# cyberlife-coder/velesdb

Measured on AMD Instinct MI355X. Metric: qps_at_recall10_1Mx768_k10, higher is better.
Workload: dtype f32; 1 GPU; 1000000x768 f32 cosine, k=10, exact distance sweep + fused GPU top-k (BASELINE configs[1]); 1024 queries/step, 1024 queries per corpus pass (sweep_topk_gemm_bf16_pp<dot, WIDE> over normalised bf16 images of rows and queries (cosine; ping-po; rows=1000000, dim=768, k=10, parallelism=replicas x1 (query stream split, no collective)

## Files before the change

velesdb_amd/csrc/select_stage.hip:

```cpp
#include <algorithm>
#include <array>
#include <cstdio>
#include <cstdlib>
#include <cstring>
#include <string>
#include <vector>

#include "vdb_probe_env.hpp"
#include "vdb_select_stage.hpp"
#include "vdb_wide.hpp"

namespace vdb {

static inline uint32_t opt_max_tile(const vdb_hip_index* ix) { return (uint32_t)opt_value(ix, VDB_OPT_MAX_QUERY_TILE); }
static inline int opt_engine(const vdb_hip_index* ix) { return (int)opt_value(ix, VDB_OPT_SWEEP_ENGINE); }
static inline int opt_selector(const vdb_hip_index* ix) { return (int)opt_value(ix, VDB_OPT_SELECTOR_LEVEL); }
static const bool g_bf16_seed = [] {
  const char* e = probe_env("VELESDB_BF16_SEED");
  return !(e && e[0] == '0');
}();
static const bool g_pool_select = [] {
  const char* e = probe_env("VELESDB_POOL_SELECT");
  return !(e && e[0] == '0');
}();
// ... 721 lines not shown
      launch_merge(true, mg, kFallbackGatherMax, st);
      ag.qcount = qcount;
      ag.qcount_max = kFallbackGatherMax;
    }
    if (!gather_all) {
      ag.part_keys = ix->s_fb_keys.as<uint64_t>();
      ag.n_rows = n;
      ag.rows = ix->rows.as<float>();
      e = launch_sweep_gemm(ix->metric, fp, ag, st, tile_needed);
      if (e != hipSuccess) return fail(VDB_ERR_HIP, std::string("exact fallback launch: ") + hipGetErrorString(e));
      MergeArgs mf{};
      mf.part_keys = ag.part_keys;
      mf.ext_ids = ix->ext_ids.as<uint64_t>();
      mf.out_ids = reinterpret_cast<uint64_t*>(sd + o_fid);
      mf.out_scores = reinterpret_cast<float*>(sd + o_fsc);
      mf.out_n = reinterpret_cast<uint32_t*>(sd + o_fn);
      mf.n_lists = fp.G;
      mf.k = k;
      mf.gate = flags;
      if (gather_ok) {
        mf.skip_cnt = qcount;
        mf.skip_le = kFallbackGatherMax;
      }
      launch_merge(true, mf, nqg, st);
      fin.fb_ids = mf.out_ids;
      fin.fb_scores = mf.out_scores;
      fin.fb_n = mf.out_n;
    }
    if (gather_ok) {
      fin.max_listed = gather_all ? 0u : kFallbackGatherMax;
      fin.g_ids = mg.out_ids;
      fin.g_scores = mg.out_scores;
      fin.g_n = mg.out_n;
    }
    launch_select_finish(fin, st);
  }
  ix->split_flags_off = o_flags;
  ix->split_flags_n = nqg;
  ix->split_flags_stream = st;
  if (ev) (void)hipEventRecord(ev->b, st);
  VDB_HIP(hipGetLastError());
  return VDB_OK;
}


static const bool g_wide_small_k = [] {
  const char* e = probe_env("VELESDB_WIDE_SMALL_K");
  return !(e && e[0] == '0');
}();
static const bool g_wide_fuse = [] {
  const char* e = probe_env("VELESDB_WIDE_FUSE");
  return !(e && e[0] == '0');
}();
int select_level_wide(vdb_hip_index* ix, uint32_t nq_left, uint32_t k, bool sq8) {
  if (opt_selector(ix) < 2 || (!sq8 && opt_engine(ix) != 1) || opt_max_tile(ix) < 128) return 0;
  if (ix->metric != VDB_COSINE && ix->metric != VDB_DOT && (sq8 || ix->metric != VDB_EUCLIDEAN)) return 0;
  if (ix->dim % 64 != 0 || ix->dim < 128 || ix->row_stride != ix->dim) return 0;
  if (k == 0 || k > kWideMaxK || ix->n_rows < kGemmBf16MinRows || ix->n_rows >= 0xFFFFFF00ull) return 0;
  if (k <= kGemmBf16MaxK && (opt_selector(ix) < 3 || !g_wide_small_k)) return 0;
  if (!sq8 && ix->metric != VDB_EUCLIDEAN && sweep_mfma_lds_bytes(1, k, ix->dim) > 160 * 1024) return 0;
  if (!sq8 && ix->metric == VDB_EUCLIDEAN && !l2_gather_fits(ix->dim, k)) return 0;
  if (!select_chunk(nq_left, sq8 ? kSelectMinQueriesSq8 : 0)) return 0;
  if (ix->sel_stats && ix->sel_stats[2] != ix->sel_seq_seen) {
    ix->sel_seq_seen = ix->sel_stats[2];
    if (ix->sel_stats[3] == 4u && (uint64_t)ix->sel_stats[0] * 16 > ix->sel_stats[1]) ix->wide_hold = 64;
  }
  if (ix->wide_hold) {
    ix->wide_hold--;
    return 0;
  }
  return 4;
}

int32_t brute_wide_dev(vdb_hip_index* ix, const float* d_q, uint64_t q_stride, uint32_t nqg, uint32_t k, uint64_t* d_ids, float* d_scores,
                       uint32_t* d_n, hipStream_t st, bool sq8) {
  const bool cosn = !sq8 && cosine_normalised(ix);
  const bool l2 = !sq8 && ix->metric == VDB_EUCLIDEAN;
  const int sel_metric = (cosn || l2) ? VDB_DOT : ix->metric;
  int32_t rc = sq8 ? ensure_sq8_select(ix, st) : (l2 ? ensure_l2_select(ix, st) : (cosn ? ensure_cosn(ix, st) : ensure_sel16(ix, st)));
  if (rc != VDB_OK) return rc;
  const uint32_t dim_a = ix->dim + 64, dim_s = ix->dim + 4;
  const uint16_t* img_rows = sq8 ? ix->sq8_img.as<uint16_t>()
                                 : (l2 ? ix->l2_img.as<uint16_t>() : (cosn ? ix->cosn_img.as<uint16_t>() : ix->rows_bf16.as<uint16_t>()));
  const uint64_t img_stride = l2 ? (uint64_t)dim_a : ((cosn || sq8) ? (uint64_t)ix->dim : ix->bf16_stride);
  const DevBuf& rho_buf = sq8 ? ix->sq8_rho : (l2 ? ix->l2_rho : (cosn ? ix->cosn_rho : ix->bf16_rho));
  const float* sel_norms = sq8 ? ix->sq8_nrm.as<float>() : ix->norms.as<float>();
  DevBuf& list_buf = sq8 ? ix->s_part_cnt : ix->s_fb_keys;
  const uint32_t sel_dim = l2 ? dim_a : ix->dim;
  ix->last_select_level = 4;
  ix->last_kernels |= VDB_KERNEL_SELECT_BF16;
  const uint8_t* alive = ix->any_dead ? ix->alive.as<uint8_t>() : nullptr;
  const uint32_t n = (uint32_t)ix->n_rows, dim = ix->dim;
  static const uint32_t g_small_seed_rows = [] {
    const char* e = probe_env("VELESDB_WIDE_SEED_ROWS");
    const long v = e ? atol(e) : 0;
    return v >= 1024 && v <= (long)kWideSeedRows ? (uint32_t)v / 256u * 256u : kSplitSeedRows;
  }();
  const uint32_t R0 = std::min<uint32_t>(k <= kWideSmallSeedMaxK ? g_small_seed_rows : kWideSeedRows, n), ngrp = (R0 + 15) / 16;
  GemmSchedule sch;
  {
    static const std::array<uint32_t, 3> mult = [] {
      std::array<uint32_t, 3> m{1, 4, 16};
      if (const char* e = probe_env("VELESDB_WIDE_STEPS")) {
        unsigned a = 0, b = 0, c = 0;
        const int got = sscanf(e, "%u,%u,%u", &a, &b, &c);
        m = {got >= 1 ? a : 0u, got >= 2 ? b : 0u, got >= 3 ? c : 0u};
      }
      return m;
    }();
    const uint32_t head[3] = {mult[0], mult[1], mult[2]};
    gemm_schedule(nqg, 0, n, ix->n_cus, head, 0, &sch);
  }
  int g_nqt = 3;
  while (g_nqt > 1 && sweep_mfma_lds_bytes(g_nqt, k, dim) > 160 * 1024) g_nqt--;
  const int g_waves = g_nqt >= 2 ? kMfmaWaves2 : kMfmaWaves1;
  const uint32_t g_B = l2 ? 8u : (uint32_t)g_nqt * 16;
  const uint32_t ntiles16 = (n + 15) / 16;
  const int g_blocks = l2 ? blocks_for(ix, 8, (n + 7) / 8)
                          : (int)std::max<int64_t>(1, std::min<int64_t>(((int64_t)ntiles16 + g_waves - 1) / g_waves, (int64_t)ix->n_cus));
  size_t off = 0;
  auto take = [&](size_t bytes) {
    const size_t o = off;
    off = (off + bytes + 15) & ~(size_t)15;
    return o;
  };
  const size_t o_tau = take((size_t)nqg * 8), o_delta = take((size_t)nqg * 4), o_qn = take((size_t)nqg * 4), o_rho = take((size_t)nqg * 4),
               o_cnt = take((size_t)nqg * 4), o_state = take((size_t)nqg * 4), o_flags = take((size_t)nqg * 4 + 16), o_qmap = take((size_t)nqg * 8),
               o_gid = take((size_t)nqg * k * 8), o_gsc = take((size_t)nqg * k * 4), o_gn = take((size_t)nqg * 4), o_nmax = take(16),
               o_extra = take((size_t)nqg * 4);
  hipError_t e;
  if ((e = ix->s_seed.reserve(off, false, st)) != hipSuccess || (e = list_buf.reserve((size_t)nqg * kWideCap * 8, false, st)) != hipSuccess ||
      (e = ix->s_part_keys.reserve((size_t)nqg * ngrp * 8, false, st)) != hipSuccess ||
      (!sq8 && (e = ix->s_part_cnt.reserve((size_t)nqg * g_blocks * k * 8, false, st)) != hipSuccess) ||
      (e = ix->s_misc.reserve(((size_t)nqg + 256) * img_stride * 2 + (l2 ? (size_t)nqg * dim_s * 4 + 16 : 0), false, st)) != hipSuccess)
    return fail(VDB_ERR_OOM, "wide selection scratch");
  unsigned char* sd = ix->s_seed.as<unsigned char>();
  uint16_t* q16 = ix->s_misc.as<uint16_t>();
  float* qnorms = reinterpret_cast<float*>(sd + o_qn);
  float* rho_q = rho_buf.p ? reinterpret_cast<float*>(sd + o_rho) : nullptr;
  uint32_t* flags = reinterpret_cast<uint32_t*>(sd + o_flags);
  uint32_t* qcount = flags + nqg;
  uint32_t* qmap = reinterpret_cast<uint32_t*>(sd + o_qmap);
  uint32_t* qslot = qmap + nqg;
  uint32_t* norm_max = reinterpret_cast<uint32_t*>(sd + o_nmax);
  EventPair* ev = next_events(ix);
  if (ev) (void)hipEventRecord(ev->a, st);
  if (l2) {
    float* qaug = reinterpret_cast<float*>(ix->s_misc.as<unsigned char>() + ((((size_t)nqg + 256) * img_stride * 2 + 15) & ~(size_t)15));
    launch_l2_augment_queries(d_q, q_stride, q16, dim_a, qaug, dim_s, nqg, dim, st);
    if (rho_q) launch_query_round_error(d_q, q_stride, rho_q, nqg, dim, st);
    PrepArgs pq{};
    pq.rows = d_q;
    pq.norms = qnorms;
    pq.row_stride = q_stride;
    pq.n_rows = nqg;
    pq.dim = dim;
    pq.words = ix->words;
    launch_prep_rows(pq, st);
    VDB_HIP(hipMemsetAsync(flags, 0, (size_t)nqg * 4 + 16, st));
  } else if (cosn) launch_seln_prep_queries(d_q, q_stride, q16, img_stride, qnorms, rho_q, flags, nqg + 4, nqg, dim, st);
  else launch_sel16_prep_queries(d_q, q_stride, q16, img_stride, qnorms, rho_q, flags, nqg + 4, nqg, dim, st);
  if (nqg % 256u) VDB_HIP(hipMemsetAsync(q16 + (size_t)nqg * img_stride, 0, (size_t)256 * img_stride * 2, st));
  if (ix->metric == VDB_DOT || l2) launch_max_norm(sel_norms, n, norm_max, st);
  WideArgs wa{};
  wa.keys = list_buf.as<uint64_t>();
  wa.eps_extra = sq8 ? 1.5e-4f : 0.0f;
  wa.cnt = reinterpret_cast<uint32_t*>(sd + o_cnt);
  wa.state = reinterpret_cast<uint32_t*>(sd + o_state);
  wa.tau = reinterpret_cast<uint64_t*>(sd + o_tau);
  wa.delta = reinterpret_cast<float*>(sd + o_delta);
  wa.qnorms = qnorms;
  wa.rho_q = rho_q;
  wa.rho_max_bits = rho_q ? rho_buf.as<uint32_t>() : nullptr;
  wa.norm_max_bits = norm_max;
  wa.extra = l2 ? reinterpret_cast<float*>(sd + o_extra) : nullptr;
  wa.cap = kWideCap;
  wa.k = k;
  wa.dim = dim;
  launch_seed_scores_bf16(sel_metric, img_rows, img_stride, sel_norms, alive, q16, img_stride, qnorms, ix->s_part_keys.as<uint64_t>(), R0,
                          nqg, sel_dim, st);
  if (l2) launch_wide_seed_l2(wa, ix->s_part_keys.as<uint64_t>(), ngrp, dim_a, nqg, st);
  else launch_wide_seed(ix->metric, wa, ix->s_part_keys.as<uint64_t>(), ngrp, nqg, st);
  for (int j = 0; j < sch.n_launch; j++) {
    EventPair* evs = next_sel_events(ix);
    if (evs) (void)hipEventRecord(evs->a, st);
    e = launch_sweep_gemm_bf16_wide(sel_metric, sch.bp[j], img_rows, img_stride, sel_norms, alive, q16, img_stride, wa.tau, wa.keys, wa.cnt,
                                    wa.cap, sel_dim, nqg, st, qnorms);
    if (evs) (void)hipEventRecord(evs->b, st);
    if (e != hipSuccess) return fail(VDB_ERR_HIP, std::string("wide selection launch: ") + hipGetErrorString(e));
    if (j + 1 < sch.n_launch || l2 || sq8 || !g_wide_fuse) launch_wide_reseed(wa, nqg, st);
  }
  WideOutArgs wo{};
  wo.rows = ix->rows.as<float>();
  wo.norms = ix->norms.as<float>();
  wo.queries = d_q;
  wo.ext_ids = ix->ext_ids.as<uint64_t>();
  wo.out_ids = d_ids;
  wo.out_scores = d_scores;
  wo.out_n = d_n;
  wo.flags = flags;
  wo.qcount = qcount;
  wo.qmap = qmap;
  wo.qslot = qslot;
  wo.row_stride = ix->row_stride;
  wo.q_stride = q_stride;
  wo.dim_pad = (dim + 127) / 128 * 128;
  if (sq8) {
    wo.sq8_codes = ix->sq8_codes.as<uint8_t>();
    wo.sq8_min = ix->sq8_min.as<float>();
    wo.sq8_max = ix->sq8_max.as<float>();
    wo.sq8_nsq = ix->sq8_nsq.as<float>();
    wo.sq8_stride = ix->sq8_stride;
    launch_wide_rerank_sq8(ix->metric, wa, wo, nqg, st);
    SelectFinishArgs fq{};
    fq.flags = flags;
    fq.qcount = qcount;
    fq.qslot = qslot;
    fq.out_ids = d_ids;
    fq.out_scores = d_scores;
    fq.out_n = d_n;
    fq.nq = nqg;
    fq.k = k;
    if (ix->sel_stats) {
      fq.stats_host = ix->sel_stats;
      fq.stats_seq = ++ix->sel_seq;
      fq.stats_level = 4u;
    }
    const int32_t rf = sq8_fallback_flagged(ix, d_q, q_stride, nqg, k, qmap, fq, st);
    if (rf != VDB_OK) return rf;
    ix->split_flags_off = o_flags;
    ix->split_flags_n = nqg;
    ix->split_flags_stream = st;
    if (ev) (void)hipEventRecord(ev->b, st);
    VDB_HIP(hipGetLastError());
    return VDB_OK;
  }
  static const bool g_wide_stamps = [] {
    const char* e = probe_env("VELESDB_WIDE_STAMPS");
    return e && e[0] == '1';
  }();
// ... 90 lines not shown
```

velesdb_amd/csrc/sweep_gemm_bf16.hip:

```cpp
#include <algorithm>

#include "vdb_probe_env.hpp"
#include "vdb_device.hpp"
#include "vdb_kernels.hpp"

namespace vdb {

typedef float f32x4 __attribute__((ext_vector_type(4)));
typedef __bf16 bf16x8 __attribute__((ext_vector_type(8)));
typedef __attribute__((address_space(3))) void* lds_ptr_t;
typedef __attribute__((address_space(3))) uint32_t lds_u32_t;

constexpr int kG16BM = 256, kG16BN = 256, kG16Waves = 8;
constexpr int kG16Cap = 12;
constexpr int kG16Queue = 39;
#ifndef VDB_G16_DUMP_MAX_LANES
#define VDB_G16_DUMP_MAX_LANES 6
#endif
constexpr int kG16DumpMaxLanes = VDB_G16_DUMP_MAX_LANES;
static_assert(kG16Queue == 39, "g16_protocol.inc keeps two hot lanes' 64 accumulators in queue entries 8 .. 39");
static_assert(kG16Queue <= 64 && kG16Queue >= 32, "the finish pass takes one queue entry per lane; one hot lane's 32 elements fit");
constexpr size_t kOffCand = 131072, kOffTauk = kOffCand + (size_t)kG16BN * kG16Cap * 8, kOffCnts = kOffTauk + kG16BN * 8,
                 kOffQn = kOffCnts + kG16BN * 4, kOffVns = kOffQn + kG16BN * 4, kOffFlags = kOffVns + kG16BM * 4,
                 kOffQueue = kOffFlags + 16,
                 kQueueBytes = 368,
                
                 kG16Lds = kOffQueue + kG16Waves * kQueueBytes;
static_assert(kG16Lds <= 160 * 1024, "LDS budget");
static_assert((size_t)(kG16Queue + 1) * 8 + kG16Queue + 4 <= 364 + 4 && (size_t)(kG16Queue + 1) * 8 + kG16Queue <= 364, "queue layout");

struct Bf16GemmArgs {
  const uint16_t* rows;
  const float* norms;
  const uint8_t* alive;
  const uint16_t* queries;
  const uint64_t* tau0;
  uint64_t* part_keys;
  uint64_t row_stride, q_stride;
  uint32_t n_rows, dim, nq, k;
  uint32_t KT, G, nqt, qper;
  uint32_t row_tile0;
  uint32_t list_stride, list_off;
  const float* qnorms;
  uint64_t* blk_tau;
  const float* qnorms_half;
  unsigned long long* dbg;
  uint64_t* wide_keys;
  uint32_t* wide_cnt;
  uint32_t wide_cap;
};

__device__ __forceinline__ uint32_t lane_now() {
  uint32_t l;
  asm volatile("v_mbcnt_lo_u32_b32 %0, -1, 0\n\tv_mbcnt_hi_u32_b32 %0, -1, %0" : "=v"(l));
  return l;
}

__device__ __forceinline__ void mfma_bf16_inplace(f32x4& c, const f32x4& a, const f32x4& b) {
  asm volatile("v_mfma_f32_16x16x32_bf16 %0, %1, %2, %0" : "+v"(c) : "v"(a), "v"(b));
}
__device__ __forceinline__ void mfma_bf16_first(f32x4& c, const f32x4& a, const f32x4& b) {
  asm volatile("v_mfma_f32_16x16x32_bf16 %0, %1, %2, 0" : "=&v"(c) : "v"(a), "v"(b));
}
__device__ __forceinline__ void mfma_drain() { asm volatile("s_nop 15\n\ts_nop 15" ::: "memory"); }

typedef int i32x4 __attribute__((ext_vector_type(4)));
__device__ __forceinline__ void glds_b128(const i32x4& rsrc, uint32_t voff, uint32_t soff, uint32_t lds_addr) {
  asm volatile("s_mov_b32 m0, %3\n\ts_nop 3\n\tbuffer_load_dwordx4 %0, %1, %2 offen lds"
               :
               : "v"(voff), "s"(rsrc), "s"(soff), "s"(lds_addr)
               : "m0");
}
__device__ __forceinline__ i32x4 make_rsrc(const void* base, uint32_t num_records = 0x7FFFFFFFu) {
  const uint64_t b = reinterpret_cast<uint64_t>(base);
  return i32x4{(int)(uint32_t)b, (int)((uint32_t)(b >> 32) & 0xFFFFu), (int)num_records, 0x00020000};
}
__device__ __forceinline__ i32x4 make_rsrc_uniform(const void* base, uint32_t num_records = 0x7FFFFFFFu) {
  const uint64_t b = reinterpret_cast<uint64_t>(base);
  const uint32_t lo = (uint32_t)__builtin_amdgcn_readfirstlane((int)(uint32_t)b);
  const uint32_t hi = (uint32_t)__builtin_amdgcn_readfirstlane((int)(uint32_t)(b >> 32));
  return i32x4{(int)lo, (int)(hi & 0xFFFFu), __builtin_amdgcn_readfirstlane((int)num_records), 0x00020000};
}
__device__ __forceinline__ uint32_t a_tile_records(uint32_t n_rows, uint32_t rt, uint32_t kt, uint64_t row_stride) {
  const uint64_t left = (uint64_t)(n_rows - rt * (uint32_t)kG16BM) * row_stride * 2u - (uint64_t)kt * 128u;
  return (uint32_t)(left < 0x7FFFFFFFull ? left : 0x7FFFFFFFull);
}
__device__ __forceinline__ uint32_t norm_records(uint32_t n_rows, uint32_t rt) {
  return min(n_rows - rt * (uint32_t)kG16BM, (uint32_t)kG16BM) * 4u;
}
__device__ __forceinline__ void wait_glds() { asm volatile("s_waitcnt vmcnt(0)" ::: "memory"); }

template <int METRIC, bool SPLIT>
__global__ __launch_bounds__(512, 2) void sweep_topk_gemm_bf16_glds(Bf16GemmArgs a) {
  constexpr bool HIB = true;
  constexpr bool WIDE = false;
  constexpr int BM = kG16BM, BN = kG16BN, WAVES = kG16Waves, CAP = kG16Cap, QCAP = kG16Queue;
  extern __shared__ __attribute__((aligned(16))) unsigned char smem[];
  uint64_t* cand = reinterpret_cast<uint64_t*>(smem + kOffCand);
  uint64_t* tauk = reinterpret_cast<uint64_t*>(smem + kOffTauk);
  uint32_t* cnts = reinterpret_cast<uint32_t*>(smem + kOffCnts);
  float* qn = reinterpret_cast<float*>(smem + kOffQn);
  float* vns = reinterpret_cast<float*>(smem + kOffVns);
// ... 162 lines not shown
  __syncthreads();
  for (uint32_t rt = rt_first; rt < ntiles; rt += a.G) {
    VDB_G16_STEP(0, true);
    __syncthreads();
    for (uint32_t kt = 1; kt + 1 < a.KT; kt++) {
      VDB_G16_STEP(kt, false);
      __syncthreads();
    }
    VDB_G16_STEP(a.KT - 1, false);
    const bool more = it < total;
#define VDB_G16_ACC_F(V) (V)
#include "g16_quicktest.inc"
    if constexpr (METRIC == kHamming || METRIC == kJaccard) {
#include "g16_quicktest_bits.inc"
    } else {
#include "g16_quicktest_dense.inc"
    }
#define VDB_G16_ACC_ELEM(X, A) asm volatile("v_mov_b32 %0, %1" : "=v"(X) : "v"(A))
#define VDB_G16_NO_DUMP 1
#include "g16_protocol.inc"
#undef VDB_G16_NO_DUMP
#undef VDB_G16_ACC_ELEM
#undef VDB_G16_ACC_F
  }
#undef VDB_G16_STEP
#undef VDB_G16_ADVANCE
#undef VDB_G16_GLDS
#undef VDB_G16_REQ
#include "g16_writeout.inc"
}

template <bool FP4>
__device__ __forceinline__ void mfma_accv(f32x4& c, const f32x4& a, const f32x4& b) {
  if (FP4)
    asm volatile("v_mfma_scale_f32_16x16x128_f8f6f4 %0, %1, %2, %0, %3, %3 op_sel_hi:[0,0,0] cbsz:4 blgp:4" : "+v"(c) : "v"(a), "v"(b), "v"(0x7F7F7F7Fu));
  else
    asm volatile("v_mfma_f32_16x16x32_bf16 %0, %1, %2, %0" : "+v"(c) : "v"(a), "v"(b));
}
template <bool FP4>
__device__ __forceinline__ void mfma_accv_first(f32x4& c, const f32x4& a, const f32x4& b) {
  if (FP4)
    asm volatile("v_mfma_scale_f32_16x16x128_f8f6f4 %0, %1, %2, 0, %3, %3 op_sel_hi:[0,0,0] cbsz:4 blgp:4" : "=&v"(c) : "v"(a), "v"(b), "v"(0x7F7F7F7Fu));
  else
    asm volatile("v_mfma_f32_16x16x32_bf16 %0, %1, %2, 0" : "=&v"(c) : "v"(a), "v"(b));
}
template <int OFF>
__device__ __forceinline__ void lds_frag_read(f32x4& dst, uint32_t addr) {
  asm volatile("ds_read_b128 %0, %1 offset:%2" : "=v"(dst) : "v"(addr), "n"(OFF));
}
__device__ __forceinline__ void pp_barrier_reads_done() { asm volatile("s_waitcnt lgkmcnt(0)\n\ts_barrier" ::: "memory"); }
__device__ __forceinline__ void pp_barrier() { asm volatile("s_barrier" ::: "memory"); }
__device__ __forceinline__ void pp_wait_dma6() { asm volatile("s_waitcnt vmcnt(6)" ::: "memory"); }

template <int METRIC, bool FP4 = false, bool WIDE = false>
__global__ __launch_bounds__(512, 2) void sweep_topk_gemm_bf16_pp(Bf16GemmArgs a) {
  static_assert(FP4 == (METRIC == kHamming || METRIC == kJaccard), "the four-bit instance serves the bit metrics, the bf16 instance Cosine / DotProduct");
  constexpr bool HIB = METRIC != kHamming;
  constexpr int BM = kG16BM, BN = kG16BN, WAVES = kG16Waves, CAP = kG16Cap, QCAP = kG16Queue;
  extern __shared__ __attribute__((aligned(16))) unsigned char smem[];
  uint64_t* cand = reinterpret_cast<uint64_t*>(smem + kOffCand);
  uint64_t* tauk = reinterpret_cast<uint64_t*>(smem + kOffTauk);
  uint32_t* cnts = reinterpret_cast<uint32_t*>(smem + kOffCnts);
  float* qn = reinterpret_cast<float*>(smem + kOffQn);
  float* vns = reinterpret_cast<float*>(smem + kOffVns);
  volatile lds_u32_t* flags = (volatile lds_u32_t*)(lds_ptr_t)(smem + kOffFlags);

  const int tid = (int)threadIdx.x;
  const int lane = tid & 63;
  const int wib = __builtin_amdgcn_readfirstlane(tid >> 6);
  const int wr = wib >> 2, wq = wib & 3;
  uint64_t* wq_keys = reinterpret_cast<uint64_t*>(smem + kOffQueue + (size_t)wib * kQueueBytes);
  uint8_t* wq_qs = reinterpret_cast<uint8_t*>(wq_keys + QCAP + 1);

  const uint32_t bid = blockIdx.x;
  const uint32_t xcd = bid & 7u, slot_id = bid >> 3;
  const uint32_t qt = slot_id % a.nqt;
  const uint32_t g = (slot_id / a.nqt) * 8u + xcd;
  const uint32_t q0 = qt * a.qper;
  const uint32_t nq_t = min(a.qper, a.nq - q0);
  const uint32_t k = a.k;
  const uint16_t* queries = a.queries + (size_t)q0 * a.q_stride;

  if (tid < BN) {
    cnts[tid] = 0;
    tauk[tid] = ((uint32_t)tid < nq_t && a.tau0) ? a.tau0[q0 + tid] : kKeyInvalid;
    qn[tid] = 0.0f;
  }
  if (tid < 4) flags[tid] = 0u;
  __syncthreads();
  if (a.qnorms) {
    if ((uint32_t)tid < nq_t) qn[tid] = a.qnorms[q0 + tid];
  } else if (a.qnorms_half) {
    if ((uint32_t)tid < nq_t) qn[tid] = a.qnorms_half[q0 + tid];
  } else {
    for (uint32_t b = wib; b < nq_t; b += WAVES) {
      const uint16_t* qp = queries + (size_t)b * a.q_stride;
      float nacc = 0.0f;
      for (uint32_t c = lane; c * 4 < a.dim; c += 64)
#pragma unroll
        for (int e = 0; e < 4; e++) {
          const uint32_t i = c * 4 + e;
          if (i < a.dim) {
            const float x = __uint_as_float((uint32_t)qp[i] << 16);
            nacc = __builtin_fmaf(x, x, nacc);
          }
        }
// ... 85 lines not shown
    } \
  } while (0)
  uint32_t c = 0;
  if (total) {
    VDB_PP_REQ_A(0, rt_first, 0, 0);
    VDB_PP_REQ_A(1, rt_first, 0, 0);
    VDB_PP_REQ_B(0, 0, 0);
    VDB_PP_REQ_B(1, 0, 0);
    VDB_PP_NEXT2();
    VDB_PP_REQ_B(0, kt2, 1);
    VDB_PP_REQ_A(0, rt2, kt2, 1);
    VDB_PP_REQ_A(1, rt2, kt2, 1);
    VDB_PP_NEXT2();
    pp_wait_dma6();
  }
  pp_barrier();
  if (total) VDB_PP_READ_A(a0v, 0, 0);
  if (wr == 1) pp_barrier();
#ifndef VDB_PP_STAMP
#define VDB_PP_STAMP 0
#endif
#ifndef VDB_PP_STAMP_METRIC
#define VDB_PP_STAMP_METRIC kCosine
#endif
#if VDB_PP_STAMP
  const bool st_on = a.dbg != nullptr && blockIdx.x == 8u && (wib == 0 || wib == 4) && METRIC == VDB_PP_STAMP_METRIC;
  uint32_t st_acc[28] = {0, 0, 0, 0, 0, 0, 0, 0, 0, 0, 0, 0, 0, 0, 0, 0, 0, 0, 0, 0, 0, 0, 0, 0, 0, 0, 0, 0};
  uint32_t st_last = 0;
#define VDB_PP_STAMP_AT(SLOT) do { \
    if (st_on) { \
      uint64_t t_; \
      asm volatile("s_memtime %0\n\ts_waitcnt lgkmcnt(0)" : "=s"(t_)::"memory"); \
      st_acc[SLOT] += (uint32_t)t_ - st_last; \
      st_last = (uint32_t)t_; \
    } \
  } while (0)
#define VDB_PP_STAMP_ISSUE(SLOT) do { if (VDB_PP_STAMP >= 2) VDB_PP_STAMP_AT(SLOT); } while (0)
#define VDB_PP_STAMP_COUNT(SLOT) do { if (st_on) st_acc[SLOT] += 1u; } while (0)
#define VDB_PP_STAMP_ADD(SLOT, N) do { if (st_on) st_acc[SLOT] += (uint32_t)(N); } while (0)
#else
#define VDB_PP_STAMP_AT(SLOT) do { } while (0)
#define VDB_PP_STAMP_ISSUE(SLOT) do { } while (0)
#endif
#define VDB_PP_LPART(READS, REQS) do { \
    READS; \
    REQS; \
  } while (0)
#define VDB_PP_KTILE(FIRST, LAST) do { \
    const uint32_t buf = c & 1u; \
     \
    VDB_PP_LPART(VDB_PP_READ_B(buf), VDB_PP_REQ_B(1, kt1, buf ^ 1u)); \
    if ((FIRST) && wib == 0)  \
      glds_b128(make_rsrc_uniform(reinterpret_cast<const unsigned char*>(a.norms) + (size_t)rt * BM * 4, norm_records(a.n_rows, rt)), lane_now() * 16u, 0u, lds0 + (uint32_t)kOffVns); \
    VDB_PP_STAMP_ISSUE(3); \
    pp_barrier_reads_done(); \
    VDB_PP_STAMP_AT(0); \
    VDB_PP_MFMA(a0v, 0, 0, FIRST); \
    VDB_PP_STAMP_AT(1); \
    pp_barrier(); \
    VDB_PP_STAMP_AT(2); \
     \
    VDB_PP_LPART(VDB_PP_READ_A(a1v, 4, buf), VDB_PP_REQ_B(0, kt2, buf)); \
    VDB_PP_STAMP_ISSUE(3); \
    pp_barrier_reads_done(); \
    VDB_PP_STAMP_AT(0); \
    VDB_PP_MFMA(a0v, 0, 2, FIRST); \
    VDB_PP_STAMP_AT(1); \
    pp_barrier(); \
    VDB_PP_STAMP_AT(2); \
     \
    VDB_PP_REQ_A(0, rt2, kt2, buf); \
    VDB_PP_STAMP_ISSUE(7); \
    pp_wait_dma6(); \
    pp_barrier_reads_done(); \
    VDB_PP_STAMP_AT(4); \
    VDB_PP_MFMA(a1v, 4, 2, FIRST); \
    VDB_PP_STAMP_AT(5); \
    pp_barrier(); \
    VDB_PP_STAMP_AT(6); \
     \
     \
    VDB_PP_LPART(if (!(LAST)) VDB_PP_READ_A(a0v, 0, buf ^ 1u), VDB_PP_REQ_A(1, rt2, kt2, buf)); \
    VDB_PP_STAMP_ISSUE(7); \
    pp_wait_dma6(); \
    pp_barrier_reads_done(); \
    VDB_PP_STAMP_AT(4); \
    VDB_PP_MFMA(a1v, 4, 0, FIRST); \
    VDB_PP_STAMP_AT(5); \
    pp_barrier(); \
    VDB_PP_STAMP_AT(6); \
    VDB_PP_NEXT2(); \
    c++; \
  } while (0)

#if VDB_PP_STAMP
  if (st_on) {
    uint64_t t_;
    asm volatile("s_memtime %0\n\ts_waitcnt lgkmcnt(0)" : "=s"(t_)::"memory");
    st_last = (uint32_t)t_;
  }
#endif
  for (uint32_t rt = rt_first; rt < ntiles; rt += a.G) {
    VDB_PP_KTILE(true, false);
    for (uint32_t kt = 1; kt + 1 < a.KT; kt++) VDB_PP_KTILE(false, false);
    VDB_PP_KTILE(false, true);
    const bool more = c < total;
    if (wr == 0) pp_barrier();
    VDB_PP_STAMP_AT(11);
#define VDB_G16_ACC_F(V) (V)
#include "g16_quicktest.inc"
    if constexpr (METRIC == kHamming || METRIC == kJaccard) {
#include "g16_quicktest_bits.inc"
    } else {
#include "g16_quicktest_dense.inc"
    }
    VDB_PP_STAMP_AT(10);
#define VDB_G16_ACC_ELEM(X, A) asm volatile("v_mov_b32 %0, %1" : "=v"(X) : "v"(A))
#include "g16_protocol.inc"
#undef VDB_G16_ACC_ELEM
#undef VDB_G16_ACC_F
    VDB_PP_LANE();
    VDB_PP_READ_A(a0v, 0, c & 1u);
    if (more && wr == 1) pp_barrier();
    VDB_PP_STAMP_AT(8);
  }
#undef VDB_PP_KTILE
#undef VDB_PP_LANE
#undef VDB_PP_NEXT2
#undef VDB_PP_MFMA
#undef VDB_PP_READ_B
#undef VDB_PP_READ_A
#undef VDB_PP_REQ_B
#undef VDB_PP_REQ_A
  asm volatile("s_waitcnt vmcnt(0)" ::: "memory");
#if VDB_PP_STAMP
  if (st_on && lane_now() == 0) {
    st_acc[9] = c;
    unsigned long long* d = a.dbg + (size_t)(wib == 0 ? 0 : 1) * 28;
    for (int i = 0; i < 28; i++) d[i] = st_acc[i];
  }
#endif
#include "g16_writeout.inc"
}

__global__ __launch_bounds__(256) void query_norms_bf16_kernel(const uint16_t* q16, uint64_t q_stride, float* out, uint32_t nq, uint32_t dim) {
  const uint32_t lane = threadIdx.x & 63u, b = blockIdx.x * 4u + (threadIdx.x >> 6);
  if (b >= nq) return;
  const uint16_t* qp = q16 + (size_t)b * q_stride;
  float nacc = 0.0f;
  for (uint32_t c = lane; c * 4 < dim; c += 64)
#pragma unroll
    for (int e = 0; e < 4; e++) {
      const uint32_t i = c * 4 + e;
      if (i < dim) {
        const float x = __uint_as_float((uint32_t)qp[i] << 16);
        nacc = __builtin_fmaf(x, x, nacc);
      }
    }
  const float n = sqrtf(butterfly_all(nacc));
  if (lane == 0) out[b] = n;
}
void launch_query_norms_bf16(const uint16_t* q16, uint64_t q_stride, float* out, uint32_t nq, uint32_t dim, hipStream_t st) {
  hipLaunchKernelGGL(query_norms_bf16_kernel, dim3((nq + 3) / 4), dim3(256), 0, st, q16, q_stride, out, nq, dim);
}

template <bool HIB>
__global__ __launch_bounds__(256) void seed_tau_kernel(const uint64_t* ids, const float* scores, const uint32_t* n, uint64_t* tau0,
                                                       uint64_t* list, uint32_t list_stride, uint32_t nq, uint32_t k) {
  const uint32_t q = blockIdx.x * 256 + threadIdx.x;
  if (q >= nq) return;
  const uint32_t c = min(n[q], k);
  uint64_t t = kKeyInvalid;
  if (c >= k && k > 0) t = make_key<HIB>(scores[(size_t)q * k + k - 1], (uint32_t)ids[(size_t)q * k + k - 1]) + 1ull;
// ... 41 lines not shown
  static bool done = false;
  if (!done) {
    hipError_t e = hipFuncSetAttribute(reinterpret_cast<const void*>(&sweep_topk_gemm_bf16_pp<METRIC>),
                                       hipFuncAttributeMaxDynamicSharedMemorySize, 160 * 1024);
    if (e != hipSuccess) return e;
    done = true;
  }
  hipLaunchKernelGGL((sweep_topk_gemm_bf16_pp<METRIC>), dim3(blocks), dim3(512), kG16Lds, st, a);
  return hipGetLastError();
}

template <int METRIC>
static hipError_t launch_g16_wide(const Bf16GemmArgs& a, int blocks, hipStream_t st) {
  static bool done = false;
  if (!done) {
    hipError_t e = hipFuncSetAttribute(reinterpret_cast<const void*>(&sweep_topk_gemm_bf16_pp<METRIC, false, true>),
                                       hipFuncAttributeMaxDynamicSharedMemorySize, 160 * 1024);
    if (e != hipSuccess) return e;
    done = true;
  }
  hipLaunchKernelGGL((sweep_topk_gemm_bf16_pp<METRIC, false, true>), dim3(blocks), dim3(512), kG16Lds, st, a);
  return hipGetLastError();
}

template <int METRIC>
static hipError_t launch_g16_fp4(const Bf16GemmArgs& a, int blocks, hipStream_t st) {
  static bool done = false;
  if (!done) {
    hipError_t e = hipFuncSetAttribute(reinterpret_cast<const void*>(&sweep_topk_gemm_bf16_pp<METRIC, true>),
                                       hipFuncAttributeMaxDynamicSharedMemorySize, 160 * 1024);
    if (e != hipSuccess) return e;
    done = true;
  }
  hipLaunchKernelGGL((sweep_topk_gemm_bf16_pp<METRIC, true>), dim3(blocks), dim3(512), kG16Lds, st, a);
  return hipGetLastError();
}

template <int METRIC, bool SPLIT>
static hipError_t launch_g16(const Bf16GemmArgs& a, int blocks, hipStream_t st) {
  static bool done = false;
  if (!done) {
    hipError_t e = hipFuncSetAttribute(reinterpret_cast<const void*>(&sweep_topk_gemm_bf16_glds<METRIC, SPLIT>),
                                       hipFuncAttributeMaxDynamicSharedMemorySize, 160 * 1024);
    if (e != hipSuccess) return e;
    done = true;
  }
  hipLaunchKernelGGL((sweep_topk_gemm_bf16_glds<METRIC, SPLIT>), dim3(blocks), dim3(512), kG16Lds, st, a);
  return hipGetLastError();
}

hipError_t launch_sweep_gemm_bf16_wide(int metric, const Bf16GemmPlan& p, const uint16_t* rows16, uint64_t row_stride, const float* norms,
                                       const uint8_t* alive, const uint16_t* queries16, uint64_t q_stride, const uint64_t* tau0,
                                       uint64_t* wide_keys, uint32_t* wide_cnt, uint32_t wide_cap, uint32_t dim, uint32_t nq, hipStream_t st,
                                       const float* qnorms) {
  Bf16GemmArgs a{};
  a.rows = rows16;
  a.norms = norms;
  a.alive = alive;
  a.queries = queries16;
  a.tau0 = tau0;
  a.row_stride = row_stride;
  a.q_stride = q_stride;
  a.n_rows = p.row_hi;
  a.row_tile0 = p.row_lo / kG16BM;
  a.dim = dim;
  a.nq = nq;
  a.k = kGemmBf16MaxK;
  a.KT = dim / 64;
  a.G = p.G;
  a.nqt = p.nqt;
  a.qper = p.qper;
  a.qnorms = qnorms;
  a.wide_keys = wide_keys;
  a.wide_cnt = wide_cnt;
  a.wide_cap = wide_cap;
#if VDB_PP_STAMP
  a.dbg = pp_stamp_dbg();
#endif
  return metric == kCosine ? launch_g16_wide<kCosine>(a, p.blocks, st) : launch_g16_wide<kDot>(a, p.blocks, st);
}

hipError_t launch_sweep_gemm_bf16_glds(int metric, const Bf16GemmPlan& p, const uint16_t* rows16, uint64_t row_stride,
                                       const float* norms, const uint8_t* alive, const uint16_t* queries16, uint64_t q_stride,
                                       const uint64_t* tau0, uint64_t* part_keys, uint32_t list_stride, uint32_t list_off,
                                       uint32_t dim, uint32_t nq, uint32_t k, hipStream_t st, bool split, const float* qnorms,
                                       uint64_t* blk_tau, const float* qnorms_half) {
  Bf16GemmArgs a{};
  a.rows = rows16;
  a.norms = norms;
  a.alive = alive;
  a.queries = queries16;
  a.tau0 = tau0;
  a.part_keys = part_keys;
  a.row_stride = row_stride;
  a.q_stride = q_stride;
  a.n_rows = p.row_hi;
  a.row_tile0 = p.row_lo / kG16BM;
  a.list_stride = list_stride;
  a.list_off = list_off;
  a.dim = dim;
  a.nq = nq;
  a.k = k;
  a.KT = split ? dim / 32 : dim / 64;
  a.G = p.G;
  a.nqt = p.nqt;
  a.qper = p.qper;
  a.qnorms = qnorms;
  a.blk_tau = blk_tau;
  a.qnorms_half = qnorms_half;
#if VDB_PP_STAMP
  a.dbg = pp_stamp_dbg();
#endif
  if (metric == kHamming) return launch_g16_fp4<kHamming>(a, p.blocks, st);
  if (metric == kJaccard) return launch_g16_fp4<kJaccard>(a, p.blocks, st);
  if (split)
    return metric == kCosine ? launch_g16<kCosine, true>(a, p.blocks, st) : launch_g16<kDot, true>(a, p.blocks, st);
  if (pingpong_enabled()) return metric == kCosine ? launch_g16_pp<kCosine>(a, p.blocks, st) : launch_g16_pp<kDot>(a, p.blocks, st);
  return metric == kCosine ? launch_g16<kCosine, false>(a, p.blocks, st) : launch_g16<kDot, false>(a, p.blocks, st);
}

}
```

velesdb_amd/csrc/sweep_wide.hip:

```cpp
#include <algorithm>

#include "vdb_device.hpp"
#include "vdb_kernels.hpp"
#include "vdb_wide.hpp"
#include "vdb_block_select.hpp"

namespace vdb {

__device__ __forceinline__ float wide_eps(uint32_t dim, const float* rho_q, const uint32_t* rho_max_bits, uint32_t q, float extra = 0.0f) {
  const float acc = 16.0f * (float)dim * 5.9604645e-8f;
  if (!rho_q || !rho_max_bits) return 2.0f * 3.90625e-3f * 1.002f + 1.6e-5f + acc + extra;
  const float rm = __uint_as_float(*rho_max_bits), rq = rho_q[q];
  return (rm + rq + 3.0f * rm * rq) * 1.002f + acc + 4e-6f + extra;
}

__device__ __forceinline__ uint64_t wide_tau_key(float s_k, float delta, bool* ok, float extra = 0.0f) {
  const float lowered = s_k - 2.0f * delta * 1.01f - extra - fabsf(s_k) * 1e-6f;
  *ok = lowered == lowered && fabsf(lowered) < 3.0e38f;
  return make_key<true>(lowered, 0u);
}
__device__ __forceinline__ uint64_t wide_tau_closed() { return make_key<true>(3.0e38f, 0u); }

template <int METRIC>
__global__ __launch_bounds__(256) void wide_seed_kernel(WideArgs a, const uint64_t* seed_keys, uint32_t ngrp) {
  __shared__ uint32_t hist[256];
  __shared__ uint32_t ctl[2];
  const uint32_t q = blockIdx.x, tid = threadIdx.x;
  constexpr int NPT = kWideSeedGroups / 256;
  uint64_t keys[NPT];
  uint32_t mine = 0;
#pragma unroll
  for (int j = 0; j < NPT; j++) {
    const uint32_t i = tid + 256u * (uint32_t)j;
    keys[j] = i < ngrp ? seed_keys[(size_t)q * ngrp + i] : kKeyInvalid;
    mine += keys[j] != kKeyInvalid ? 1u : 0u;
  }
  const float eps = wide_eps(a.dim, a.rho_q, a.rho_max_bits, q, a.eps_extra);
  const float d = METRIC == kCosine ? eps * 1.001f + 4e-7f : eps * 1.001f * a.qnorms[q] * __uint_as_float(*a.norm_max_bits) + 1e-30f;
  __shared__ uint32_t total;
  if (tid == 0) total = 0;
  __syncthreads();
  if (mine) atomicAdd(&total, mine);
  __syncthreads();
  const uint32_t valid = total;
  bool ok = valid >= a.k && d == d;
  uint64_t tau = wide_tau_closed();
  if (ok) {
    __shared__ uint64_t s256[256];
    const uint32_t hi = ngrp <= 256 ? block_kth_hi_256(keys[0], a.k, s256, ctl) : block_kth_hi<NPT>(keys, a.k, hist, ctl);
    tau = wide_tau_key(key_score<true>((uint64_t)hi << 32), d, &ok);
    if (!ok) tau = wide_tau_closed();
  }
  if (tid == 0) {
    a.delta[q] = d;
    a.tau[q] = tau;
    a.cnt[q] = 0;
    a.state[q] = ok ? 0u : kWideGivenUp;
  }
}

template <int NPT>
__device__ int wide_next_tau(const WideArgs& a, uint32_t raw, const uint64_t (&keys)[NPT], float delta, float extra, uint64_t old, uint32_t* hist,
                             uint32_t* ctl, uint64_t* s256, uint64_t* tau_out) {
  if (raw > a.cap) return 2;
  if (raw < a.k) return 0;
  const uint32_t hi = raw <= 256 ? block_kth_hi_256(keys[0], a.k, s256, ctl, (raw + 7u) & ~7u) : block_kth_hi<NPT>(keys, a.k, hist, ctl);
  bool ok;
  uint64_t tau = wide_tau_key(key_score<true>((uint64_t)hi << 32), delta, &ok, extra);
  if (!ok) return 2;
  if (tau > old) tau = old;
  *tau_out = tau;
  return 1;
}

__global__ __launch_bounds__(256) void wide_reseed_kernel(WideArgs a) {
  __shared__ uint32_t hist[256];
  __shared__ uint32_t ctl[2];
  __shared__ uint32_t wsum[4];
  __shared__ uint64_t s256[256];
  const uint32_t q = blockIdx.x, tid = threadIdx.x;
  const uint32_t state = a.state[q], raw = a.cnt[q];
  const float delta = a.delta[q], extra = a.extra ? a.extra[q] : 0.0f;
  const uint64_t old = a.tau[q];
  if (state & kWideGivenUp) return;
  constexpr int NPT = kWideCap / 256;
  uint64_t* list = a.keys + (size_t)q * a.cap;
  uint64_t keys[NPT];
  keys[0] = list[tid];
  if (tid >= raw) keys[0] = kKeyInvalid;
#pragma unroll
  for (int j = 1; j < NPT; j++) {
    const uint32_t i = tid + 256u * (uint32_t)j;
    keys[j] = (i < raw && i < a.cap) ? list[i] : kKeyInvalid;
  }
  uint64_t tau = 0;
  const int what = wide_next_tau<NPT>(a, raw, keys, delta, extra, old, hist, ctl, s256, &tau);
  if (what == 0) return;
  if (what == 2) {
    if (tid == 0) {
      a.state[q] |= kWideGivenUp;
      a.tau[q] = wide_tau_closed();
    }
    return;
  }
  uint32_t keep = 0;
#pragma unroll
  for (int j = 0; j < NPT; j++) keep += (keys[j] != kKeyInvalid && keys[j] < tau) ? 1u : 0u;
  uint32_t incl = keep;
  const uint32_t lane = tid & 63u, w = tid >> 6;
#pragma unroll
  for (int o = 1; o < 64; o <<= 1) {
// ... 467 lines not shown
```

velesdb_amd/csrc/vdb_wide.hpp:

```cpp
#pragma once
#include <hip/hip_runtime.h>
#include <stdint.h>

#include "vdb_gemm_schedule.hpp"

namespace vdb {

constexpr uint32_t kWideMaxK = 128;
constexpr uint32_t kWideCap = 4096;
constexpr uint32_t kWidePoolMax = 1024;
constexpr uint32_t kWideSeedRows = 16384;
constexpr uint32_t kWideSeedGroups = kWideSeedRows / 16;
constexpr uint32_t kWideSmallSeedMaxK = 32;
constexpr uint32_t kWideGivenUp = 1u;

struct WideArgs {
  uint64_t* keys;
  uint32_t* cnt;
  uint32_t* state;
  uint64_t* tau;
  float* delta;
  const float* qnorms;
  const float* rho_q;
  const uint32_t* rho_max_bits;
  const uint32_t* norm_max_bits;
  float* extra;
  uint32_t cap, k, dim;
  float eps_extra;
};
struct WideOutArgs {
  const float* rows;
  const float* norms;
  const float* queries;
  const uint64_t* ext_ids;
  uint64_t* out_ids;
  float* out_scores;
  uint32_t* out_n;
  uint32_t* flags;
  uint32_t* qcount;
  uint32_t* qmap;
  uint32_t* qslot;
  uint64_t row_stride, q_stride;
  uint32_t dim_pad;
  const uint8_t* sq8_codes;
  const float* sq8_min;
  const float* sq8_max;
  const float* sq8_nsq;
  uint64_t sq8_stride;
  unsigned long long* stamps;
};

void launch_wide_seed(int metric, const WideArgs& a, const uint64_t* seed_keys, uint32_t ngrp, uint32_t nq, hipStream_t st);
void launch_wide_reseed(const WideArgs& a, uint32_t nq, hipStream_t st);
void launch_wide_rerank(int metric, const WideArgs& a, const WideOutArgs& o, uint32_t nq, bool fuse_final_reseed, hipStream_t st);
void launch_wide_seed_l2(const WideArgs& a, const uint64_t* seed_keys, uint32_t ngrp, uint32_t dim_a, uint32_t nq, hipStream_t st);
void launch_wide_rerank_l2(const WideArgs& a, const WideOutArgs& o, uint32_t nq, hipStream_t st);
void launch_wide_rerank_sq8(int metric, const WideArgs& a, const WideOutArgs& o, uint32_t nq, hipStream_t st);
hipError_t launch_sweep_gemm_bf16_wide(int metric, const Bf16GemmPlan& p, const uint16_t* rows16, uint64_t row_stride, const float* norms,
                                       const uint8_t* alive, const uint16_t* queries16, uint64_t q_stride, const uint64_t* tau0,
                                       uint64_t* wide_keys, uint32_t* wide_cnt, uint32_t wide_cap, uint32_t dim, uint32_t nq, hipStream_t st,
                                       const float* qnorms);

}
```

Baseline: 755,500 queries/s.

## Tighten wide top-k threshold live inside the sweep kernel instead of relaunching

```diff
diff --git a/velesdb_amd/csrc/select_stage.hip b/velesdb_amd/csrc/select_stage.hip
--- a/velesdb_amd/csrc/select_stage.hip
+++ b/velesdb_amd/csrc/select_stage.hip
@@ -797,6 +797,14 @@
   const char* e = probe_env("VELESDB_WIDE_FUSE");
   return !(e && e[0] == '0');
 }();
+static const bool g_wide_live = [] {
+  const char* e = probe_env("VELESDB_WIDE_LIVE");
+  return !(e && e[0] == '0');
+}();
+static const uint32_t g_wide_ckpt = [] {
+  const char* e = probe_env("VELESDB_WIDE_CKPT");
+  return e ? (uint32_t)strtoul(e, nullptr, 0) : kWideLiveCkpt;
+}();
 int select_level_wide(vdb_hip_index* ix, uint32_t nq_left, uint32_t k, bool sq8) {
   if (opt_selector(ix) < 2 || (!sq8 && opt_engine(ix) != 1) || opt_max_tile(ix) < 128) return 0;
   if (ix->metric != VDB_COSINE && ix->metric != VDB_DOT && (sq8 || ix->metric != VDB_EUCLIDEAN)) return 0;
@@ -842,8 +850,12 @@
     return v >= 1024 && v <= (long)kWideSeedRows ? (uint32_t)v / 256u * 256u : kSplitSeedRows;
   }();
   const uint32_t R0 = std::min<uint32_t>(k <= kWideSmallSeedMaxK ? g_small_seed_rows : kWideSeedRows, n), ngrp = (R0 + 15) / 16;
+  const bool live = !l2 && !sq8 && g_wide_fuse && g_wide_live;
   GemmSchedule sch;
-  {
+  if (live) {
+    const uint32_t none[3] = {0, 0, 0};
+    gemm_schedule(nqg, 0, n, ix->n_cus, none, 0, &sch);
+  } else {
     static const std::array<uint32_t, 3> mult = [] {
       std::array<uint32_t, 3> m{1, 4, 16};
       if (const char* e = probe_env("VELESDB_WIDE_STEPS")) {
@@ -922,6 +934,7 @@
   wa.cap = kWideCap;
   wa.k = k;
   wa.dim = dim;
+  wa.clear = live ? kWideLiveMax : 0u;
   launch_seed_scores_bf16(sel_metric, img_rows, img_stride, sel_norms, alive, q16, img_stride, qnorms, ix->s_part_keys.as<uint64_t>(), R0,
                           nqg, sel_dim, st);
   if (l2) launch_wide_seed_l2(wa, ix->s_part_keys.as<uint64_t>(), ngrp, dim_a, nqg, st);
@@ -930,7 +943,7 @@
     EventPair* evs = next_sel_events(ix);
     if (evs) (void)hipEventRecord(evs->a, st);
     e = launch_sweep_gemm_bf16_wide(sel_metric, sch.bp[j], img_rows, img_stride, sel_norms, alive, q16, img_stride, wa.tau, wa.keys, wa.cnt,
-                                    wa.cap, sel_dim, nqg, st, qnorms);
+                                    wa.cap, sel_dim, nqg, st, qnorms, live ? &wa : nullptr, g_wide_ckpt);
     if (evs) (void)hipEventRecord(evs->b, st);
     if (e != hipSuccess) return fail(VDB_ERR_HIP, std::string("wide selection launch: ") + hipGetErrorString(e));
     if (j + 1 < sch.n_launch || l2 || sq8 || !g_wide_fuse) launch_wide_reseed(wa, nqg, st);
diff --git a/velesdb_amd/csrc/sweep_gemm_bf16.hip b/velesdb_amd/csrc/sweep_gemm_bf16.hip
--- a/velesdb_amd/csrc/sweep_gemm_bf16.hip
+++ b/velesdb_amd/csrc/sweep_gemm_bf16.hip
@@ -3,6 +3,7 @@
 #include "vdb_probe_env.hpp"
 #include "vdb_device.hpp"
 #include "vdb_kernels.hpp"
+#include "vdb_wide.hpp"
 
 namespace vdb {
 
@@ -48,6 +49,10 @@
   uint64_t* wide_keys;
   uint32_t* wide_cnt;
   uint32_t wide_cap;
+  uint64_t* wide_tau;
+  const float* wide_delta;
+  const uint32_t* wide_state;
+  uint32_t wide_k, wide_ckpt;
 };
 
 __device__ __forceinline__ uint32_t lane_now() {
@@ -316,6 +321,39 @@
 __device__ __forceinline__ void pp_barrier() { asm volatile("s_barrier" ::: "memory"); }
 __device__ __forceinline__ void pp_wait_dma6() { asm volatile("s_waitcnt vmcnt(6)" ::: "memory"); }
 
+__device__ __forceinline__ void wide_live_reseed(const Bf16GemmArgs& a, uint32_t qg) {
+  if (a.wide_state[qg] & kWideGivenUp) return;
+  const uint32_t raw = __hip_atomic_load(&a.wide_cnt[qg], __ATOMIC_RELAXED, __HIP_MEMORY_SCOPE_AGENT);
+  const uint32_t n = min(min(raw, a.wide_cap), kWideLiveMax);
+  if (n < a.wide_k) return;
+  const uint32_t ln = lane_now();
+  const uint64_t* list = a.wide_keys + (size_t)qg * a.wide_cap;
+  constexpr int NPT = kWideLiveMax / 64;
+  const uint32_t nj = (n + 63u) / 64u;
+  uint32_t h[NPT];
+#pragma unroll
+  for (int j = 0; j < NPT; j++) {
+    const uint32_t i = ln + 64u * (uint32_t)j;
+    h[j] = 0xFFFFFFFFu;
+    if ((uint32_t)j < nj && i < n) h[j] = (uint32_t)(__hip_atomic_load(&list[i], __ATOMIC_RELAXED, __HIP_MEMORY_SCOPE_AGENT) >> 32);
+  }
+  uint32_t pre = 0, kk = a.wide_k;
+#pragma unroll 1
+  for (int bit = 31; bit >= 8; bit--) {
+    uint32_t c0 = 0;
+#pragma unroll
+    for (int j = 0; j < NPT; j++)
+      if ((uint32_t)j < nj) c0 += (uint32_t)__popcll(__ballot((h[j] >> bit) == (pre >> bit)));
+    if (kk > c0) {
+      kk -= c0;
+      pre |= 1u << bit;
+    }
+  }
+  bool ok;
+  const uint64_t tau = wide_tau_key(key_score<true>((uint64_t)(pre | 0xFFu) << 32), a.wide_delta[qg], &ok);
+  if (ok && ln == 0) atomicMin(reinterpret_cast<unsigned long long*>(&a.wide_tau[qg]), (unsigned long long)tau);
+}
+
 template <int METRIC, bool FP4 = false, bool WIDE = false>
 __global__ __launch_bounds__(512, 2) void sweep_topk_gemm_bf16_pp(Bf16GemmArgs a) {
   static_assert(FP4 == (METRIC == kHamming || METRIC == kJaccard), "the four-bit instance serves the bit metrics, the bf16 instance Cosine / DotProduct");
@@ -507,6 +545,9 @@
     VDB_PP_LPART(VDB_PP_READ_B(buf), VDB_PP_REQ_B(1, kt1, buf ^ 1u)); \
     if ((FIRST) && wib == 0)  \
       glds_b128(make_rsrc_uniform(reinterpret_cast<const unsigned char*>(a.norms) + (size_t)rt * BM * 4, norm_records(a.n_rows, rt)), lane_now() * 16u, 0u, lds0 + (uint32_t)kOffVns); \
+    if (WIDE && (FIRST) && a.wide_tau && (wib == 1 || wib == 2))  \
+      glds_b128(make_rsrc_uniform(a.wide_tau + q0 + 128u * (uint32_t)(wib - 1), nq_t > 128u * (uint32_t)(wib - 1) ? min(nq_t - 128u * (uint32_t)(wib - 1), 128u) * 8u : 0u), \
+                lane_now() * 16u, 0u, lds0 + (uint32_t)kOffTauk + (uint32_t)(wib - 1) * 1024u); \
     VDB_PP_STAMP_ISSUE(3); \
     pp_barrier_reads_done(); \
     VDB_PP_STAMP_AT(0); \
@@ -574,6 +615,26 @@
 #include "g16_protocol.inc"
 #undef VDB_G16_ACC_ELEM
 #undef VDB_G16_ACC_F
+    if constexpr (WIDE) {
+      const uint32_t lt = a.wide_tau && more ? (rt - rt_first) / a.G + 1u : 32u;
+      if (lt < 32u && ((a.wide_ckpt >> lt) & 1u)) {
+        if (wib < 4) {
+          const uint32_t t_c = (uint32_t)wib * 64u + lane_now();
+          if (t_c < nq_t) {
+            const uint32_t ns = min(cnts[t_c], (uint32_t)CAP);
+            if (ns) {
+              const uint32_t base = atomicAdd(&a.wide_cnt[q0 + t_c], ns);
+              uint64_t* dst = a.wide_keys + (size_t)(q0 + t_c) * a.wide_cap;
+              for (uint32_t e = 0; e < ns; e++)
+                if (base + e < a.wide_cap) dst[base + e] = cand[(size_t)t_c * CAP + e];
+            }
+            cnts[t_c] = 0;
+          }
+        } else {
+          for (uint32_t b = g + a.G * (uint32_t)(wib - 4); b < nq_t; b += 4u * a.G) wide_live_reseed(a, q0 + b);
+        }
+      }
+    }
     VDB_PP_LANE();
     VDB_PP_READ_A(a0v, 0, c & 1u);
     if (more && wr == 1) pp_barrier();
@@ -721,7 +782,7 @@
 hipError_t launch_sweep_gemm_bf16_wide(int metric, const Bf16GemmPlan& p, const uint16_t* rows16, uint64_t row_stride, const float* norms,
                                        const uint8_t* alive, const uint16_t* queries16, uint64_t q_stride, const uint64_t* tau0,
                                        uint64_t* wide_keys, uint32_t* wide_cnt, uint32_t wide_cap, uint32_t dim, uint32_t nq, hipStream_t st,
-                                       const float* qnorms) {
+                                       const float* qnorms, const WideArgs* live, uint32_t live_ckpt) {
   Bf16GemmArgs a{};
   a.rows = rows16;
   a.norms = norms;
@@ -743,6 +804,13 @@
   a.wide_keys = wide_keys;
   a.wide_cnt = wide_cnt;
   a.wide_cap = wide_cap;
+  if (live) {
+    a.wide_tau = live->tau;
+    a.wide_delta = live->delta;
+    a.wide_state = live->state;
+    a.wide_k = live->k;
+    a.wide_ckpt = live_ckpt;
+  }
 #if VDB_PP_STAMP
   a.dbg = pp_stamp_dbg();
 #endif
diff --git a/velesdb_amd/csrc/sweep_wide.hip b/velesdb_amd/csrc/sweep_wide.hip
--- a/velesdb_amd/csrc/sweep_wide.hip
+++ b/velesdb_amd/csrc/sweep_wide.hip
@@ -13,13 +13,6 @@
   const float rm = __uint_as_float(*rho_max_bits), rq = rho_q[q];
   return (rm + rq + 3.0f * rm * rq) * 1.002f + acc + 4e-6f + extra;
 }
-
-__device__ __forceinline__ uint64_t wide_tau_key(float s_k, float delta, bool* ok, float extra = 0.0f) {
-  const float lowered = s_k - 2.0f * delta * 1.01f - extra - fabsf(s_k) * 1e-6f;
-  *ok = lowered == lowered && fabsf(lowered) < 3.0e38f;
-  return make_key<true>(lowered, 0u);
-}
-__device__ __forceinline__ uint64_t wide_tau_closed() { return make_key<true>(3.0e38f, 0u); }
 
 template <int METRIC>
 __global__ __launch_bounds__(256) void wide_seed_kernel(WideArgs a, const uint64_t* seed_keys, uint32_t ngrp) {
@@ -57,6 +50,7 @@
     a.cnt[q] = 0;
     a.state[q] = ok ? 0u : kWideGivenUp;
   }
+  for (uint32_t i = tid; i < a.clear; i += 256) a.keys[(size_t)q * a.cap + i] = kKeyInvalid;
 }
 
 template <int NPT>
diff --git a/velesdb_amd/csrc/vdb_wide.hpp b/velesdb_amd/csrc/vdb_wide.hpp
--- a/velesdb_amd/csrc/vdb_wide.hpp
+++ b/velesdb_amd/csrc/vdb_wide.hpp
@@ -2,6 +2,7 @@
 #include <hip/hip_runtime.h>
 #include <stdint.h>
 
+#include "vdb_device.hpp"
 #include "vdb_gemm_schedule.hpp"
 
 namespace vdb {
@@ -13,6 +14,8 @@
 constexpr uint32_t kWideSeedGroups = kWideSeedRows / 16;
 constexpr uint32_t kWideSmallSeedMaxK = 32;
 constexpr uint32_t kWideGivenUp = 1u;
+constexpr uint32_t kWideLiveMax = 1024;
+constexpr uint32_t kWideLiveCkpt = (1u << 1) | (1u << 2) | (1u << 4) | (1u << 8) | (1u << 16);
 
 struct WideArgs {
   uint64_t* keys;
@@ -26,6 +29,7 @@
   const uint32_t* norm_max_bits;
   float* extra;
   uint32_t cap, k, dim;
+  uint32_t clear;
   float eps_extra;
 };
 struct WideOutArgs {
@@ -50,6 +54,13 @@
   unsigned long long* stamps;
 };
 
+__device__ __forceinline__ uint64_t wide_tau_key(float s_k, float delta, bool* ok, float extra = 0.0f) {
+  const float lowered = s_k - 2.0f * delta * 1.01f - extra - fabsf(s_k) * 1e-6f;
+  *ok = lowered == lowered && fabsf(lowered) < 3.0e38f;
+  return make_key<true>(lowered, 0u);
+}
+__device__ __forceinline__ uint64_t wide_tau_closed() { return make_key<true>(3.0e38f, 0u); }
+
 void launch_wide_seed(int metric, const WideArgs& a, const uint64_t* seed_keys, uint32_t ngrp, uint32_t nq, hipStream_t st);
 void launch_wide_reseed(const WideArgs& a, uint32_t nq, hipStream_t st);
 void launch_wide_rerank(int metric, const WideArgs& a, const WideOutArgs& o, uint32_t nq, bool fuse_final_reseed, hipStream_t st);
@@ -59,6 +70,6 @@
 hipError_t launch_sweep_gemm_bf16_wide(int metric, const Bf16GemmPlan& p, const uint16_t* rows16, uint64_t row_stride, const float* norms,
                                        const uint8_t* alive, const uint16_t* queries16, uint64_t q_stride, const uint64_t* tau0,
                                        uint64_t* wide_keys, uint32_t* wide_cnt, uint32_t wide_cap, uint32_t dim, uint32_t nq, hipStream_t st,
-                                       const float* qnorms);
+                                       const float* qnorms, const WideArgs* live = nullptr, uint32_t live_ckpt = 0);
 
 }
```

After: 736,200 queries/s (median of 2 runs). 2.6% lower.
